# google-research/multinerf

Hardware: NVIDIA H100
Metric: train-step rays/sec @16384 rays x (64+64+32) samples (higher is better)
Workload: dtype bf16

## Files before the change

### multinerf_b200/csrc/gemm_tc.cu

```cuda
#include <cuda.h>

#include <stdlib.h>
#include <string.h>

#include <algorithm>

#include "tc_common.cuh"

namespace mnrf {

constexpr int BLOCK_M = 128;
constexpr int BLOCK_K = 64;
constexpr int A_STAGE_BYTES = BLOCK_M * BLOCK_K * 2;
constexpr int NUM_THREADS = 384;
constexpr int CS_MAX = 1024;
constexpr int gemm_stages(int bn) { return bn == 256 ? 4 : bn == 128 ? 6 : 8; }
constexpr int STAGING_BLOCK_BYTES = 64 * 128;
constexpr int staging_blocks(int mode, int bn, bool ts) {
  return !ts ? 0 : (mode == MNRF_GEMM_FWD && bn >= 128) ? 2 : 1;
}
constexpr int mask_words(int bn) { return bn >= 128 ? bn / 32 : 0; }
constexpr int MASK_BUFS = 2;
constexpr int dgrad_smem_bytes(int bn) { return 8 * bn * 4 + MASK_BUFS * BLOCK_M * mask_words(bn) * 4; }
constexpr int SIDE_SCRATCH = 96 * 8;
// ... 95 lines not shown
      const int64_t col0 = WEIGHTED ? (int64_t)m_blk * BLOCK_M : (int64_t)n_blk * COLS;
      float* out = WEIGHTED ? p.side_aw : p.bsum;
      for (int col = t; col < COLS; col += NT) {
        if (WEIGHTED && col0 + col >= p.m) break;
        float sum = 0.f;
#pragma unroll
        for (int g = 0; g < G; ++g) sum += __uint_as_float(ld_shared_u32(scratch + (g * COLS + col) * 4));
        atomicAdd(out + col0 + col, sum);
      }
    }
  }
}

enum { GK_TURN, GK_FULL, GK_MMA, GK_EPI_LOOP, GK_EPI_SYNC, GK_MASK, GK_N };
#ifdef MNRF_GEMM_CLOCKS
__device__ unsigned long long g_gemm_clk[2][GK_N];
struct GemmClk {
  long long t[GK_N] = {};
  long long last = 0;
  __device__ __forceinline__ void start() { last = clock64(); }
  __device__ __forceinline__ void tick(int k) {
    const long long now = clock64();
    t[k] += now - last;
    last = now;
  }
};
#else
struct GemmClk {
  __device__ __forceinline__ void start() {}
  __device__ __forceinline__ void tick(int) {}
};
#endif

enum { EPI_GENERIC = 0, EPI_BITS_TMA = 1, EPI_BITS_TMA_RANK1 = 2 };

template <int MODE, int NC, bool TS, int SB, bool SMOOTH, int OPS = EPI_GENERIC>
__device__ __forceinline__ void gemm_epilogue(const GemmParams& p, const CUtensorMap* tmap_c, const float (&acc)[NC / 2],
                                              int m_blk, int r0, int ncol0, int wg, uint8_t* smem_c, bool mask_tma,
                                              uint32_t m_tile, bool do_cs, uint32_t cs_lane, int& sblk, GemmClk& clk) {
  constexpr int MW = mask_words(NC);
  static_assert(OPS == EPI_GENERIC || (MODE == MNRF_GEMM_DGRAD && TS && !SMOOTH && MW > 0),
                "fixed operand sets are DGRAD epilogues of the staged store with TMA-loaded mask bits");
  constexpr bool kFixed = OPS != EPI_GENERIC;
  const bool has_rowv = kFixed ? OPS == EPI_BITS_TMA_RANK1 : p.rowv != nullptr;
  const bool has_bits = kFixed || p.maskbits != nullptr;
  const bool bits_tma = kFixed || mask_tma;
  const bool has_mask = !kFixed && p.mask != nullptr;
  const bool has_addend = !kFixed && p.addend != nullptr;
  const int lane = threadIdx.x & 31;
  const int r_in = r0 + (16 * ((threadIdx.x >> 5) & 3) + (lane >> 2));
  const int cq = 2 * (lane & 3);
  const bool leader = (threadIdx.x & 127) == 0;
  const uint32_t c_row = smem_u32(smem_c) + wg * (SB * STAGING_BLOCK_BYTES) + (r_in - r0) * 128 + (cq << 1);
  const uint32_t m_row = m_tile + r_in * (MW * 4);
  int64_t rows[2];
  bool row_ok[2];
  float rv[2] = {0.f, 0.f};
  const uint32_t* mrow[2] = {nullptr, nullptr};
#pragma unroll
  for (int h = 0; h < 2; ++h) {
    rows[h] = (int64_t)m_blk * BLOCK_M + r_in + 8 * h;
    row_ok[h] = rows[h] < p.m;
    if (MODE == MNRF_GEMM_DGRAD && row_ok[h]) {
      if (has_rowv) rv[h] = p.rowv[rows[h]];
      if (has_bits && !bits_tma)
        mrow[h] = p.maskbits + (p.mask_mod > 0 ? rows[h] % p.mask_mod : rows[h]) * p.ldmaskbits;
    }
  }
  uint32_t bits[2] = {0u, 0u};
  uint32_t mw[2] = {0u, 0u};
#pragma unroll
  for (int i = 0; i < NC / 8; ++i) {
    const int col = ncol0 + 8 * i + cq;
    const int sb = SB == 3 ? sblk : (i >> 3) & (SB - 1);
    if (TS && SB == 1 && (i & 7) == 0) {
      clk.tick(GK_EPI_LOOP);
      if (leader) tma_store_wait_read<0>();
      named_bar_sync(2 + wg, 128);
      clk.tick(GK_EPI_SYNC);
    }
    if (MODE == MNRF_GEMM_DGRAD && has_bits && (i & 3) == 0) {
#pragma unroll
      for (int h = 0; h < 2; ++h)
        mw[h] = bits_tma ? ld_shared_u32(m_row + (8 * h * MW + (i >> 2)) * 4)
                         : row_ok[h] ? __ldg(mrow[h] + (col >> 5)) : 0u;
    }
    float v[2][2];
#pragma unroll
    for (int h = 0; h < 2; ++h) { v[h][0] = acc[4 * i + 2 * h]; v[h][1] = acc[4 * i + 2 * h + 1]; }
    if (MODE == MNRF_GEMM_FWD) {
      if (p.bias) {
        const float2 b = __ldg(reinterpret_cast<const float2*>(p.bias + col));
#pragma unroll
        for (int h = 0; h < 2; ++h) { v[h][0] += b.x; v[h][1] += b.y; }
      }
      if constexpr (SMOOTH) {
#pragma unroll
        for (int h = 0; h < 2; ++h) {
          if (p.mask && row_ok[h])
            *reinterpret_cast<uint32_t*>(const_cast<__nv_bfloat16*>(p.mask) + rows[h] * p.ldmask + col) =
                pack_bf16(v[h][0], v[h][1]);
          v[h][0] = act_fwd(p.act, v[h][0]);
          v[h][1] = act_fwd(p.act, v[h][1]);
        }
      } else if (p.act == MNRF_ACT_RELU) {
#pragma unroll
        for (int h = 0; h < 2; ++h)
#pragma unroll
          for (int e = 0; e < 2; ++e) {
            v[h][e] = relu_nan(v[h][e]);
            bits[h] |= (v[h][e] > 0.f ? 1u : 0u) << ((8 * i + cq + e) & 31);
          }
      }
    } else {
      float2 cv = make_float2(0.f, 0.f);
      if (has_rowv) cv = __ldg(reinterpret_cast<const float2*>(p.colv + col));
#pragma unroll
      for (int h = 0; h < 2; ++h) {
        if (has_rowv) { v[h][0] += rv[h] * cv.x; v[h][1] += rv[h] * cv.y; }
        if constexpr (SMOOTH) {
          if (row_ok[h]) {
            const int64_t zr = p.mask_mod > 0 ? rows[h] % p.mask_mod : rows[h];
            const uint32_t zz = __ldg(reinterpret_cast<const unsigned int*>(p.mask + zr * p.ldmask + col));
            v[h][0] *= act_d1(p.act, bf16_lo(zz));
            v[h][1] *= act_d1(p.act, bf16_hi(zz));
          }
        } else if (has_bits) {
          if (!((mw[h] >> (col & 31)) & 1u)) v[h][0] = 0.f;
          if (!((mw[h] >> ((col + 1) & 31)) & 1u)) v[h][1] = 0.f;
        } else if (has_mask && row_ok[h]) {
          const uint32_t mm = __ldg(reinterpret_cast<const unsigned int*>(p.mask + rows[h] * p.ldmask + col));
          if (!(bf16_lo(mm) > 0.f)) v[h][0] = 0.f;
          if (!(bf16_hi(mm) > 0.f)) v[h][1] = 0.f;
        }
        if (has_addend && row_ok[h]) {
          const uint32_t aa = __ldg(reinterpret_cast<const unsigned int*>(p.addend + rows[h] * p.ldadd + col));
          v[h][0] += bf16_lo(aa);
          v[h][1] += bf16_hi(aa);
        }
      }
      if (do_cs) {
        const bool hi = (lane >> 2) & 1;
        const float s0 = v[0][0] + v[1][0], s1 = v[0][1] + v[1][1];
        float t = (hi ? s1 : s0) + __shfl_xor_sync(0xffffffffu, hi ? s0 : s1, 4);
        t += __shfl_xor_sync(0xffffffffu, t, 8);
        t += __shfl_xor_sync(0xffffffffu, t, 16);
        if (lane < 8) {
          const uint32_t a = cs_lane + 8 * i * 4;
          st_shared_u32(a, __float_as_uint(__uint_as_float(ld_shared_u32(a)) + t));
        }
      }
    }
#pragma unroll
    for (int h = 0; h < 2; ++h) {
      if (TS) {
        st_shared_u32(c_row + sb * STAGING_BLOCK_BYTES + h * (8 * 128) + (((i & 7) ^ ((lane >> 2) & 7)) << 4),
                      pack_bf16(v[h][0], v[h][1]));
      } else if (row_ok[h]) {
        *reinterpret_cast<uint32_t*>(reinterpret_cast<__nv_bfloat16*>(p.out) + rows[h] * p.ldc + col) =
            pack_bf16(v[h][0], v[h][1]);
      }
    }
    if (MODE == MNRF_GEMM_FWD && p.act == MNRF_ACT_RELU && p.maskbits && (i & 3) == 3) {
#pragma unroll
      for (int h = 0; h < 2; ++h) {
        bits[h] |= __shfl_xor_sync(0xffffffffu, bits[h], 1);
        bits[h] |= __shfl_xor_sync(0xffffffffu, bits[h], 2);
        if ((lane & 3) == ((i >> 2) & 3) && row_ok[h]) p.maskbits[rows[h] * p.ldmaskbits + (col >> 5)] = bits[h];
        bits[h] = 0u;
      }
    }
    if (TS && (i & 7) == 7) {
      fence_proxy_async();
      clk.tick(GK_EPI_LOOP);
      if (SB >= 2 && leader) tma_store_wait_read<SB - 2>();
      named_bar_sync(2 + wg, 128);
      if (leader) {
        tma_store_2d(tmap_c, smem_c + (wg * SB + sb) * STAGING_BLOCK_BYTES, ncol0 + 8 * (i & ~7),
                     (int)((int64_t)m_blk * BLOCK_M + r0));
        tma_store_commit();
      }
      if (SB == 3) sblk = sblk == 2 ? 0 : sblk + 1;
      clk.tick(GK_EPI_SYNC);
    }
  }
}

template <int MODE, int BN, bool TS, bool SIDE, bool SMOOTH = false>
__global__ void __launch_bounds__(NUM_THREADS, 1)
gemm_tc_kernel(const __grid_constant__ CUtensorMap tmap_a, const __grid_constant__ CUtensorMap tmap_b,
               const __grid_constant__ CUtensorMap tmap_c, const __grid_constant__ CUtensorMap tmap_m,
               const GemmParams p) {
  constexpr int STAGES = gemm_stages(BN);
  constexpr int B_STAGE = BN * BLOCK_K * 2;
  constexpr bool kWgrad = (MODE == MNRF_GEMM_WGRAD);
  constexpr bool kDgrad = (MODE == MNRF_GEMM_DGRAD);
  constexpr int NACC = BN / 2;
  constexpr int SB = staging_blocks(MODE, BN, TS);
  constexpr int MW = mask_words(BN);
  static_assert(SB < 2 || (BN / 64) % 2 == 0, "block j of every tile must use staging block j % SB");
  static_assert(!SIDE || kWgrad, "side sums are a WGRAD feature");
  static_assert(!SMOOTH || (TS && !kWgrad), "smooth activations are FWD / DGRAD epilogues of the staged store");
  extern __shared__ uint8_t smem_dyn[];
  uint8_t* smem = reinterpret_cast<uint8_t*>((reinterpret_cast<uintptr_t>(smem_dyn) + 1023) & ~uintptr_t(1023));
  uint8_t* smem_a = smem;
  uint8_t* smem_b = smem + STAGES * A_STAGE_BYTES;
  uint8_t* smem_c = smem_b + STAGES * B_STAGE;
  float* cs_s = reinterpret_cast<float*>(smem_c + 2 * SB * STAGING_BLOCK_BYTES);
  float* side_s = cs_s;
  uint32_t* mask_s = reinterpret_cast<uint32_t*>(cs_s + (kDgrad ? 8 * BN : SIDE ? SIDE_SCRATCH : 0));
  uint64_t* full_bar = reinterpret_cast<uint64_t*>(mask_s + (kDgrad ? MASK_BUFS * BLOCK_M * MW : 0));
  uint64_t* empty_bar = full_bar + STAGES;
// ... 130 lines not shown
      int sblk = 0;
      GemmClk clk;
      clk.start();
      gemm_epilogue<MODE, BN, TS, SB, SMOOTH>(p, &tmap_c, acc, m_blk, 64 * c, ncol0, c, smem_c, mask_tma,
                                              smem_u32(mask_s) + (it % MASK_BUFS) * (BLOCK_M * MW * 4), do_cs, cs_lane,
                                              sblk, clk);
      if (mask_tma) {
        __syncwarp();
        if (lane == 0) mbar_arrive(&mask_empty[it % MASK_BUFS]);
      }
      const int next = tile + (int)gridDim.x;
      if (do_cs && (next >= total_tiles || next % p.num_n_blocks != n_blk)) {
        named_bar_sync(1, 2 * 128);
        for (int j = threadIdx.x - 128; j < BN; j += 2 * 128) {
          float s = 0.f;
#pragma unroll
          for (int sw = 0; sw < 8; ++sw) {
            s += cs_s[sw * BN + j];
            cs_s[sw * BN + j] = 0.f;
          }
          atomicAdd(p.colsum + ncol0 + j, s);
        }
        named_bar_sync(1, 2 * 128);
      }
    }
    if (TS && (threadIdx.x & 127) == 0) tma_store_wait_all();
  }
}

constexpr int PP_BN = 128;
constexpr int PP_STAGES = 5;
constexpr int pp_staging_blocks(int mode) { return mode == MNRF_GEMM_DGRAD ? 3 : 2; }
constexpr int PP_MASK_BUFS = 4;
constexpr int pp_smem_bytes(int mode) {
  return PP_STAGES * (A_STAGE_BYTES + PP_BN * BLOCK_K * 2) + 2 * pp_staging_blocks(mode) * STAGING_BLOCK_BYTES +
         (mode == MNRF_GEMM_DGRAD ? PP_MASK_BUFS * BLOCK_M * mask_words(PP_BN) * 4 : 0) + 256  +
         1024 ;
}

template <int MODE, int BN, int OPS>
__global__ void __launch_bounds__(NUM_THREADS, 1)
gemm_tc_pingpong_kernel(const __grid_constant__ CUtensorMap tmap_a, const __grid_constant__ CUtensorMap tmap_b,
                        const __grid_constant__ CUtensorMap tmap_c, const __grid_constant__ CUtensorMap tmap_m,
                        const GemmParams p) {
  constexpr int STAGES = PP_STAGES;
  constexpr int B_STAGE = PP_BN * BLOCK_K * 2;
  constexpr int SUB = BN / PP_BN;
  constexpr int MW = mask_words(PP_BN);
  constexpr int SB = pp_staging_blocks(MODE);
  constexpr bool kDgrad = (MODE == MNRF_GEMM_DGRAD);
  static_assert(MODE != MNRF_GEMM_WGRAD && (BN == 128 || BN == 256), "FWD / DGRAD tiles of 128 or 256 columns");
  extern __shared__ uint8_t smem_dyn[];
  uint8_t* smem = reinterpret_cast<uint8_t*>((reinterpret_cast<uintptr_t>(smem_dyn) + 1023) & ~uintptr_t(1023));
  uint8_t* smem_a = smem;
  uint8_t* smem_b = smem + STAGES * A_STAGE_BYTES;
  uint8_t* smem_c = smem_b + STAGES * B_STAGE;
  uint32_t* mask_s = reinterpret_cast<uint32_t*>(smem_c + 2 * SB * STAGING_BLOCK_BYTES);
  uint64_t* full_bar = reinterpret_cast<uint64_t*>(mask_s + (kDgrad ? PP_MASK_BUFS * BLOCK_M * MW : 0));
  uint64_t* empty_bar = full_bar + STAGES;
  uint64_t* mask_full = empty_bar + STAGES;
  uint64_t* mask_empty = mask_full + PP_MASK_BUFS;
  uint64_t* mma_turn = mask_empty + PP_MASK_BUFS;

  const int lane = threadIdx.x & 31;
  const int wg = threadIdx.x >> 7;
  const int total_tiles = p.num_m_blocks * p.num_n_blocks;
  const int nk = p.num_k_blocks;
  const bool mask_tma = kDgrad && (OPS != EPI_GENERIC || p.mask_tma);

  if (threadIdx.x == 0) {
    prefetch_tmap(&tmap_a);
    prefetch_tmap(&tmap_b);
    prefetch_tmap(&tmap_c);
    if (mask_tma) prefetch_tmap(&tmap_m);
    for (int i = 0; i < STAGES; ++i) {
      mbar_init(&full_bar[i], 1);
      mbar_init(&empty_bar[i], 4);
    }
    for (int i = 0; i < PP_MASK_BUFS; ++i) {
      mbar_init(&mask_full[i], 1);
      mbar_init(&mask_empty[i], 4);
    }
    for (int i = 0; i < 2; ++i) mbar_init(&mma_turn[i], 4);
    fence_barrier_init();
  }
  __syncthreads();
  pdl_launch_dependents();
  pdl_wait();

  if (wg == 0) {
    setmaxnreg_dec<40>();
    if (threadIdx.x == 0) {
      uint32_t stage = 0, phase = 0;
      int it = 0;
      for (int tile = blockIdx.x; tile < total_tiles; tile += gridDim.x) {
        const int n_blk = tile % p.num_n_blocks;
        const int m_blk = tile / p.num_n_blocks;
        for (int s = 0; s < SUB; ++s, ++it) {
          const int ncol0 = n_blk * BN + s * PP_BN;
          if (mask_tma) {
            const int mb = it % PP_MASK_BUFS;
            mbar_wait(&mask_empty[mb], ((it / PP_MASK_BUFS) & 1) ^ 1, 4);
            mbar_expect_tx(&mask_full[mb], BLOCK_M * MW * 4);
            const int64_t r0 = (int64_t)m_blk * BLOCK_M;
            tma_load_2d(mask_s + mb * (BLOCK_M * MW), &tmap_m, &mask_full[mb], ncol0 / 32,
                        (int)(p.mask_mod > 0 ? r0 % p.mask_mod : r0));
          }
          for (int kb = 0; kb < nk; ++kb) {
            mbar_wait(&empty_bar[stage], phase ^ 1, 1);
            mbar_expect_tx(&full_bar[stage], A_STAGE_BYTES + B_STAGE);
            tma_load_2d(smem_a + stage * A_STAGE_BYTES, &tmap_a, &full_bar[stage], kb * BLOCK_K, m_blk * BLOCK_M);
            tma_load_2d(smem_b + stage * B_STAGE, &tmap_b, &full_bar[stage], kb * BLOCK_K, ncol0);
            if (++stage == STAGES) { stage = 0; phase ^= 1; }
          }
        }
      }
    }
  } else {
    setmaxnreg_inc<232>();
    const int c = wg - 1;
    float acc[2][64];
    int sblk = 0;
    GemmClk clk;
    clk.start();
    for (int it = c; ; it += 2) {
      const int tile = blockIdx.x + (it / SUB) * (int)gridDim.x;
      if (tile >= total_tiles) break;
      const int s = it % SUB;
      const int n_blk = tile % p.num_n_blocks;
      const int m_blk = tile / p.num_n_blocks;
      const int ncol0 = n_blk * BN + s * PP_BN;
      const uint32_t slot = (uint32_t)it * (uint32_t)nk;
      uint32_t stage = slot % STAGES, phase = (slot / STAGES) & 1;
      clk.tick(GK_EPI_LOOP);
      if (it > 0) mbar_wait(&mma_turn[c], ((it - 1) >> 1) & 1, 7);
      clk.tick(GK_TURN);
      int prev = -1;
      fence_acc(acc[0]);
      fence_acc(acc[1]);
      for (int kb = 0; kb < nk; ++kb) {
        mbar_wait(&full_bar[stage], phase, 3);
        clk.tick(GK_FULL);
        const uint32_t sa = smem_u32(smem_a + stage * A_STAGE_BYTES);
        const uint32_t sb = smem_u32(smem_b + stage * B_STAGE);
        wgmma_fence();
#pragma unroll
        for (int k = 0; k < BLOCK_K / WGMMA_K; ++k) {
          const uint64_t bdesc = make_smem_desc(sb + k * (WGMMA_K * 2), 0, 1024);
#pragma unroll
          for (int g = 0; g < 2; ++g)
            Wgmma<PP_BN, 0, 0>::mma(acc[g], make_smem_desc(sa + g * (64 * 128) + k * (WGMMA_K * 2), 0, 1024), bdesc,
                                    (kb > 0 || k > 0) ? 1u : 0u);
        }
        wgmma_commit();
        wgmma_wait<1>();
        if (prev >= 0 && lane == 0) mbar_arrive(&empty_bar[prev]);
        prev = (int)stage;
        if (++stage == STAGES) { stage = 0; phase ^= 1; }
        clk.tick(GK_MMA);
      }
      if (blockIdx.x + ((it + 1) / SUB) * (int)gridDim.x < total_tiles) {
        __syncwarp();
        if (lane == 0) mbar_arrive(&mma_turn[c ^ 1]);
      }
      wgmma_wait<0>();
      fence_acc(acc[0]);
      fence_acc(acc[1]);
      if (prev >= 0 && lane == 0) mbar_arrive(&empty_bar[prev]);
      clk.tick(GK_MMA);

      const uint32_t m_base = smem_u32(mask_s) + (it % PP_MASK_BUFS) * (BLOCK_M * MW * 4);
      if (mask_tma) mbar_wait(&mask_full[it % PP_MASK_BUFS], (it / PP_MASK_BUFS) & 1, 5);
      clk.tick(GK_MASK);
#pragma unroll 1
      for (int g = 0; g < 2; ++g) {
        gemm_epilogue<MODE, PP_BN, true, SB, false, OPS>(p, &tmap_c, acc[0], m_blk, 64 * g, ncol0, c, smem_c, mask_tma,
                                                         m_base, false, 0, sblk, clk);
#pragma unroll
        for (int e = 0; e < 64; ++e) acc[0][e] = acc[1][e];
      }
      if (mask_tma) {
        __syncwarp();
        if (lane == 0) mbar_arrive(&mask_empty[it % PP_MASK_BUFS]);
      }
    }
    if ((threadIdx.x & 127) == 0) tma_store_wait_all();
#ifdef MNRF_GEMM_CLOCKS
    clk.tick(GK_EPI_SYNC);
    if (blockIdx.x == 0 && (threadIdx.x & 127) == 0)
      for (int k = 0; k < GK_N; ++k) atomicAdd(&g_gemm_clk[c][k], (unsigned long long)clk.t[k]);
#endif
  }
}

template <int MODE, int BN, int OPS = EPI_GENERIC>
static int launch_gemm_tc_pingpong(int grid, const CUtensorMap& ta, const CUtensorMap& tb, const CUtensorMap& tc,
                                   const CUtensorMap& tm, const GemmParams& p, cudaStream_t stream) {
  constexpr int kSmem = pp_smem_bytes(MODE);
  static_assert(kSmem <= 232448, "shared memory budget");
  return launch_tc<gemm_tc_pingpong_kernel<MODE, BN, OPS>>(grid, NUM_THREADS, kSmem, stream, ta, tb, tc, tm, p);
}

template <int BN>
static int launch_dgrad_pingpong(int ops, int grid, const CUtensorMap& ta, const CUtensorMap& tb, const CUtensorMap& tc,
                                 const CUtensorMap& tm, const GemmParams& p, cudaStream_t stream) {
  switch (ops) {
    case EPI_BITS_TMA:
      return launch_gemm_tc_pingpong<MNRF_GEMM_DGRAD, BN, EPI_BITS_TMA>(grid, ta, tb, tc, tm, p, stream);
    case EPI_BITS_TMA_RANK1:
      return launch_gemm_tc_pingpong<MNRF_GEMM_DGRAD, BN, EPI_BITS_TMA_RANK1>(grid, ta, tb, tc, tm, p, stream);
  }
  return launch_gemm_tc_pingpong<MNRF_GEMM_DGRAD, BN>(grid, ta, tb, tc, tm, p, stream);
}

template <int MODE, int BN, bool TS, bool SIDE, bool SMOOTH = false>
static int launch_gemm_tc(int grid, const CUtensorMap& ta, const CUtensorMap& tb, const CUtensorMap& tc,
                          const CUtensorMap& tm, const GemmParams& p, cudaStream_t stream) {
  constexpr int kSmem = smem_bytes(MODE, BN, TS, SIDE);
  static_assert(kSmem <= 232448, "shared memory budget");
  return launch_tc<gemm_tc_kernel<MODE, BN, TS, SIDE, SMOOTH>>(grid, NUM_THREADS, kSmem, stream, ta, tb, tc, tm, p);
}

int gemm_tc_smooth_launch(int mode, int block_n, int grid, const CUtensorMap& ta, const CUtensorMap& tb,
                          const CUtensorMap& tc, const GemmParams& p, cudaStream_t stream);

#ifndef MNRF_GEMM_TC_SMOOTH_UNIT
static int pick_block_n(int n) {
  const int cands[] = {256, 128, 64, 32, 16};
  for (int c : cands)
    if (n % c == 0) return c;
  return 0;
}

static int gemm_tc_plan(const mnrf_gemm_desc* d, const mnrf_bf16* a, const mnrf_bf16* b, const float* bias,
                        const float* colv, const mnrf_bf16* mask, const uint32_t* maskbits, const float* colsum,
                        const mnrf_bf16* addend, const void* out, const float* bsum, const float* side_w,
                        const float* side_aw, const mnrf_bf16* z, int64_t ldz, mnrf_gemm_instance* plan,
                        GemmParams* p) {
  MNRF_CHECK(d->mode == MNRF_GEMM_WGRAD || d->k % BLOCK_K == 0,
             "mnrf_gemm(tc): reduction length %d must be a multiple of %d", d->k, BLOCK_K);
  MNRF_CHECK(d->lda % 8 == 0 && d->ldb % 8 == 0 && ((uintptr_t)a % 16) == 0 && ((uintptr_t)b % 16) == 0,
             "mnrf_gemm(tc): operands must be 16-byte aligned with ld %% 8 == 0");
  const int block_n = pick_block_n(d->n);
  MNRF_CHECK(block_n > 0, "mnrf_gemm(tc): N=%d must be a multiple of 16", d->n);
  if (d->mode == MNRF_GEMM_WGRAD)
// ... 15 lines not shown
    MNRF_CHECK(!maskbits && !mask, "mnrf_gemm(tc): a smooth activation takes z, not a ReLU mask");
    MNRF_CHECK(d->mode == MNRF_GEMM_FWD || z, "mnrf_gemm(tc): the DGRAD of a smooth activation needs z");
    MNRF_CHECK(!z || (ldz % 2 == 0 && ((uintptr_t)z % 4) == 0), "mnrf_gemm(tc): z must be 4-byte aligned");
  }
  if (bias) MNRF_CHECK(((uintptr_t)bias % 8) == 0, "mnrf_gemm(tc): bias must be 8-byte aligned");
  if (colv) MNRF_CHECK(((uintptr_t)colv % 8) == 0, "mnrf_gemm(tc): colv must be 8-byte aligned");
  const int workers = mnrf_num_sms();
  const int num_m_blocks = (int)((d->m + BLOCK_M - 1) / BLOCK_M);
  const int num_n_blocks = d->n / block_n;
  const int num_k_blocks = (d->k + BLOCK_K - 1) / BLOCK_K;
  int num_splits = 1;
  if (d->mode == MNRF_GEMM_WGRAD) {
    const int out_tiles = num_m_blocks * num_n_blocks;
    const int max_splits = std::min(std::max(1, (2 * workers) / out_tiles), num_k_blocks);
    int splits = max_splits;
    for (int sp = 1; sp <= max_splits; ++sp) {
      const int items = out_tiles * sp;
      const int rounds = (items + workers - 1) / workers;
      if (items * 100 >= rounds * workers * 95) { splits = sp; break; }
    }
    num_splits = splits;
  }
  const int kblocks_per_split = (num_k_blocks + num_splits - 1) / num_splits;
  num_splits = (num_k_blocks + kblocks_per_split - 1) / kblocks_per_split;
  if (d->mode != MNRF_GEMM_WGRAD) {
    MNRF_CHECK(d->ldc % 2 == 0 && ((uintptr_t)out % 4) == 0, "mnrf_gemm(tc): bf16 output must be 4-byte aligned");
    if (mask) MNRF_CHECK(d->ldmask % 2 == 0 && ((uintptr_t)mask % 4) == 0, "mnrf_gemm(tc): mask must be 4-byte aligned");
  } else {
    MNRF_CHECK(d->ldc % 2 == 0 && ((uintptr_t)out % 8) == 0, "mnrf_gemm(tc): fp32 output must be 8-byte aligned");
  }
  const bool ts = d->mode != MNRF_GEMM_WGRAD && block_n >= 64 && ((uintptr_t)out % 16) == 0 && d->ldc % 8 == 0;
  MNRF_CHECK(!smooth || ts, "mnrf_gemm(tc): a smooth activation needs N %% 64 == 0 and a 16-byte aligned output "
             "with a row pitch that is a multiple of 8");
  const bool mask_tma = d->mode == MNRF_GEMM_DGRAD && maskbits && mask_words(block_n) > 0 && d->ldmaskbits % 4 == 0 &&
                        ((uintptr_t)maskbits % 16) == 0 && (d->mask_mod == 0 || d->mask_mod % BLOCK_M == 0);
  const bool pingpong = d->mode != MNRF_GEMM_WGRAD && ts && d->n % PP_BN == 0 && !smooth && !colsum;
  int epilogue = EPI_GENERIC;
  if (pingpong && d->mode == MNRF_GEMM_DGRAD && mask_tma && !mask && !addend)
    epilogue = colv ? EPI_BITS_TMA_RANK1 : EPI_BITS_TMA;
  const int tiles = num_m_blocks * num_n_blocks * num_splits;
  plan->block_n = block_n;
  plan->staged = ts;
  plan->mask_tma = mask_tma;
  plan->smooth = smooth;
  plan->side = side;
  plan->splits = num_splits;
  plan->tiles = tiles;
  plan->grid = std::min(tiles, workers);
  plan->pingpong = pingpong;
  plan->epilogue = epilogue;
  p->num_m_blocks = num_m_blocks;
  p->num_n_blocks = num_n_blocks;
  p->num_k_blocks = num_k_blocks;
  p->num_splits = num_splits;
  p->kblocks_per_split = kblocks_per_split;
  return 0;
}

template <int MODE>
static int launch_register_store(int block_n, int grid, const CUtensorMap& ta, const CUtensorMap& tb,
                                 const CUtensorMap& tc, const CUtensorMap& tm, const GemmParams& p,
                                 cudaStream_t stream) {
  switch (block_n) {
    case 256: return launch_gemm_tc<MODE, 256, false, false>(grid, ta, tb, tc, tm, p, stream);
    case 128: return launch_gemm_tc<MODE, 128, false, false>(grid, ta, tb, tc, tm, p, stream);
    case 64: return launch_gemm_tc<MODE, 64, false, false>(grid, ta, tb, tc, tm, p, stream);
    case 32: return launch_gemm_tc<MODE, 32, false, false>(grid, ta, tb, tc, tm, p, stream);
    case 16: return launch_gemm_tc<MODE, 16, false, false>(grid, ta, tb, tc, tm, p, stream);
  }
  set_error("mnrf_gemm(tc): no register-store instance at BN=%d", block_n);
  return 1;
}

static int launch_gemm_tc_plan(int mode, const mnrf_gemm_instance& plan, const CUtensorMap& ta, const CUtensorMap& tb,
                               const CUtensorMap& tc, const CUtensorMap& tm, const GemmParams& p,
                               cudaStream_t stream) {
  const int bn = plan.block_n, grid = plan.grid;
  const bool fwd = mode == MNRF_GEMM_FWD;
  if (plan.pingpong) {
    if (bn == 256)
      return fwd ? launch_gemm_tc_pingpong<MNRF_GEMM_FWD, 256>(grid, ta, tb, tc, tm, p, stream)
                 : launch_dgrad_pingpong<256>(plan.epilogue, grid, ta, tb, tc, tm, p, stream);
    if (bn == 128)
      return fwd ? launch_gemm_tc_pingpong<MNRF_GEMM_FWD, 128>(grid, ta, tb, tc, tm, p, stream)
                 : launch_dgrad_pingpong<128>(plan.epilogue, grid, ta, tb, tc, tm, p, stream);
  } else if (plan.smooth) {
    return gemm_tc_smooth_launch(mode, bn, grid, ta, tb, tc, p, stream);
  } else if (mode == MNRF_GEMM_WGRAD) {
    if (bn == 256)
      return plan.side ? launch_gemm_tc<MNRF_GEMM_WGRAD, 256, false, true>(grid, ta, tb, tc, tm, p, stream)
                       : launch_gemm_tc<MNRF_GEMM_WGRAD, 256, false, false>(grid, ta, tb, tc, tm, p, stream);
    if (bn == 128)
      return plan.side ? launch_gemm_tc<MNRF_GEMM_WGRAD, 128, false, true>(grid, ta, tb, tc, tm, p, stream)
                       : launch_gemm_tc<MNRF_GEMM_WGRAD, 128, false, false>(grid, ta, tb, tc, tm, p, stream);
    if (bn == 64)
      return plan.side ? launch_gemm_tc<MNRF_GEMM_WGRAD, 64, false, true>(grid, ta, tb, tc, tm, p, stream)
                       : launch_gemm_tc<MNRF_GEMM_WGRAD, 64, false, false>(grid, ta, tb, tc, tm, p, stream);
  } else if (!plan.staged) {
    return fwd ? launch_register_store<MNRF_GEMM_FWD>(bn, grid, ta, tb, tc, tm, p, stream)
               : launch_register_store<MNRF_GEMM_DGRAD>(bn, grid, ta, tb, tc, tm, p, stream);
  } else if (bn == 64) {
    return fwd ? launch_gemm_tc<MNRF_GEMM_FWD, 64, true, false>(grid, ta, tb, tc, tm, p, stream)
               : launch_gemm_tc<MNRF_GEMM_DGRAD, 64, true, false>(grid, ta, tb, tc, tm, p, stream);
  } else if (!fwd) {
    if (bn == 256) return launch_gemm_tc<MNRF_GEMM_DGRAD, 256, true, false>(grid, ta, tb, tc, tm, p, stream);
    if (bn == 128) return launch_gemm_tc<MNRF_GEMM_DGRAD, 128, true, false>(grid, ta, tb, tc, tm, p, stream);
  }
  set_error("mnrf_gemm(tc): no kernel instance for mode %d, BN=%d, staged %d, side sums %d", mode, bn, plan.staged,
            plan.side);
  return 1;
}

int gemm_tc_launch(const mnrf_gemm_desc* d, const mnrf_bf16* a, const mnrf_bf16* b, const float* bias,
                   const float* rowv, const float* colv, const mnrf_bf16* mask, uint32_t* maskbits,
                   float* colsum, const mnrf_bf16* addend, void* out, cudaStream_t stream, float* bsum,
                   const float* side_w, float* side_aw, mnrf_bf16* z, int64_t ldz) {
  mnrf_gemm_instance plan;
// ... 5 lines not shown
  const bool ts = plan.staged;
  p.mode = d->mode; p.act = d->act; p.m = d->m; p.n = d->n; p.k = d->k;
  p.ldc = d->ldc; p.ldmask = d->ldmask;
  p.bias = bias; p.rowv = rowv; p.colv = colv;
  p.mask = reinterpret_cast<const __nv_bfloat16*>(mask);
  p.out = out;
  p.maskbits = maskbits;
  p.ldmaskbits = d->ldmaskbits;
  p.mask_mod = d->mask_mod;
  p.addend = reinterpret_cast<const __nv_bfloat16*>(addend);
  p.ldadd = d->ldadd;
  p.colsum = colsum;
  p.bsum = bsum; p.side_w = side_w; p.side_aw = side_aw;
  if (plan.smooth) {
    p.mask = reinterpret_cast<const __nv_bfloat16*>(z);
    p.ldmask = ldz;
  }
  p.mask_tma = plan.mask_tma;
  CUtensorMap ta, tb, tc;
  if (d->mode != MNRF_GEMM_WGRAD) {
    if (make_tmap(&ta, a, d->m, d->k, d->lda, BLOCK_K, BLOCK_M)) return 1;
    if (make_tmap(&tb, b, d->n, d->k, d->ldb, BLOCK_K, plan.pingpong ? PP_BN : block_n)) return 1;
  } else {
    if (make_tmap(&ta, a, d->k, d->m, d->lda, 64, BLOCK_K)) return 1;
    if (make_tmap(&tb, b, d->k, d->n, d->ldb, 64, BLOCK_K)) return 1;
  }
  if (ts) {
    if (make_tmap(&tc, out, d->m, d->n, d->ldc, 64, 64)) return 1;
  } else {
    tc = tb;
  }
  CUtensorMap tm = tb;
  if (p.mask_tma &&
      make_tmap(&tm, maskbits, d->mask_mod > 0 ? d->mask_mod : d->m, d->n / 32, d->ldmaskbits,
                mask_words(plan.pingpong ? PP_BN : block_n), BLOCK_M, CU_TENSOR_MAP_DATA_TYPE_UINT32, 4,
                CU_TENSOR_MAP_SWIZZLE_NONE))
    return 1;
  if (plan.grid == 0) return 0;
  if (int rc = launch_gemm_tc_plan(d->mode, plan, ta, tb, tc, tm, p, stream)) return rc;
  MNRF_LAUNCH_CHECK();
  return 0;
}
#endif

}

#ifndef MNRF_GEMM_TC_SMOOTH_UNIT
extern "C" int mnrf_gemm_plan(const mnrf_gemm_desc* d, const mnrf_bf16* a, const mnrf_bf16* b, const float* bias,
                              const float* rowv, const float* colv, const mnrf_bf16* mask, const uint32_t* maskbits,
                              const float* colsum, const mnrf_bf16* addend, const mnrf_bf16* z, int64_t ldz,
                              const void* out, const float* bsum, const float* side_w, const float* side_aw,
                              mnrf_gemm_instance* plan) {
  MNRF_CHECK(d && plan, "mnrf_gemm_plan: null pointer");
  MNRF_CHECK((rowv == nullptr) == (colv == nullptr), "mnrf_gemm: rowv and colv come together");
  MNRF_CHECK(!mask || d->mask_mod == 0, "mnrf_gemm: mask_mod applies to maskbits and z, not to a bf16 mask");
  mnrf::GemmParams p;
  return mnrf::gemm_tc_plan(d, a, b, bias, colv, mask, maskbits, colsum, addend, out, bsum, side_w, side_aw, z, ldz,
                            plan, &p);
}

#ifdef MNRF_GEMM_CLOCKS
extern "C" int mnrf_gemm_clocks(unsigned long long* out) {
  unsigned long long zero[2 * mnrf::GK_N] = {};
  if (cudaDeviceSynchronize() != cudaSuccess) return 1;
  if (cudaMemcpyFromSymbol(out, mnrf::g_gemm_clk, sizeof(zero)) != cudaSuccess) return 1;
  return cudaMemcpyToSymbol(mnrf::g_gemm_clk, zero, sizeof(zero)) != cudaSuccess;
}
// ... 3 lines not shown
```

### multinerf_b200/csrc/tc_common.cuh

```cuda
#pragma once

#include <cuda.h>
#include <stdlib.h>

#include "common.cuh"
#include "wgmma.cuh"

namespace mnrf {

constexpr int WGMMA_K = 16;

__device__ __forceinline__ uint32_t smem_u32(const void* p) {
  return static_cast<uint32_t>(__cvta_generic_to_shared(p));
}
__device__ __forceinline__ void mbar_init(uint64_t* bar, uint32_t count) {
  asm volatile("mbarrier.init.shared::cta.b64 [%0], %1;" ::"r"(smem_u32(bar)), "r"(count));
}
__device__ __forceinline__ void mbar_expect_tx(uint64_t* bar, uint32_t bytes) {
  asm volatile("mbarrier.arrive.expect_tx.shared::cta.b64 _, [%0], %1;" ::"r"(smem_u32(bar)), "r"(bytes) : "memory");
}
__device__ __forceinline__ void mbar_arrive(uint64_t* bar) {
  asm volatile("mbarrier.arrive.shared::cta.b64 _, [%0];" ::"r"(smem_u32(bar)) : "memory");
}
__device__ __forceinline__ bool mbar_try_wait(uint64_t* bar, uint32_t parity) {
// ... 2 lines not shown
      "{\n"
      ".reg .pred p;\n"
      "mbarrier.try_wait.parity.shared::cta.b64 p, [%1], %2;\n"
      "selp.u32 %0, 1, 0, p;\n"
      "}\n"
      : "=r"(ok) : "r"(smem_u32(bar)), "r"(parity) : "memory");
  return ok != 0;
}
__device__ __forceinline__ void mbar_wait(uint64_t* bar, uint32_t parity, int tag) {
  (void)tag;
  if (mbar_try_wait(bar, parity)) return;
  const long long t0 = clock64();
  while (!mbar_try_wait(bar, parity)) {
    if (clock64() - t0 > 4000000000LL) __trap();
  }
}
__device__ __forceinline__ void fence_barrier_init() {
  asm volatile("fence.mbarrier_init.release.cluster;" ::: "memory");
}
__device__ __forceinline__ void fence_proxy_async() {
  asm volatile("fence.proxy.async.shared::cta;" ::: "memory");
}
__device__ __forceinline__ void tma_load_2d(void* smem_dst, const CUtensorMap* map, uint64_t* bar,
                                            int c0, int c1) {
  asm volatile(
      "cp.async.bulk.tensor.2d.shared::cluster.global.mbarrier::complete_tx::bytes [%0], [%1, {%3, %4}], [%2];"
      :: "r"(smem_u32(smem_dst)), "l"(reinterpret_cast<uint64_t>(map)), "r"(smem_u32(bar)), "r"(c0), "r"(c1)
      : "memory");
}
__device__ __forceinline__ void tma_prefetch_2d(const CUtensorMap* map, int c0, int c1) {
  asm volatile("cp.async.bulk.prefetch.tensor.2d.L2.global.tile [%0, {%1, %2}];"
               :: "l"(reinterpret_cast<uint64_t>(map)), "r"(c0), "r"(c1) : "memory");
}
__device__ __forceinline__ void tma_store_2d(const CUtensorMap* map, const void* smem_src, int c0, int c1) {
  asm volatile("cp.async.bulk.tensor.2d.global.shared::cta.bulk_group [%0, {%2, %3}], [%1];"
               :: "l"(reinterpret_cast<uint64_t>(map)), "r"(smem_u32(smem_src)), "r"(c0), "r"(c1) : "memory");
}
__device__ __forceinline__ void tma_store_commit() { asm volatile("cp.async.bulk.commit_group;" ::: "memory"); }
template <int N>
__device__ __forceinline__ void tma_store_wait_read() {
  asm volatile("cp.async.bulk.wait_group.read %0;" ::"n"(N) : "memory");
}
__device__ __forceinline__ void tma_store_wait_all() { asm volatile("cp.async.bulk.wait_group 0;" ::: "memory"); }
__device__ __forceinline__ void prefetch_tmap(const CUtensorMap* map) {
  asm volatile("prefetch.tensormap [%0];" ::"l"(reinterpret_cast<uint64_t>(map)) : "memory");
}
__device__ __forceinline__ void st_shared_u32(uint32_t addr, uint32_t v) {
  asm volatile("st.shared.b32 [%0], %1;" ::"r"(addr), "r"(v) : "memory");
}
__device__ __forceinline__ uint32_t ld_shared_u32(uint32_t addr) {
  uint32_t v;
  asm volatile("ld.shared.b32 %0, [%1];" : "=r"(v) : "r"(addr) : "memory");
  return v;
}
__device__ __forceinline__ uint4 ld_shared_v4(uint32_t addr) {
  uint4 v;
  asm volatile("ld.shared.v4.b32 {%0, %1, %2, %3}, [%4];"
               : "=r"(v.x), "=r"(v.y), "=r"(v.z), "=r"(v.w) : "r"(addr) : "memory");
  return v;
}
__device__ __forceinline__ void named_bar_sync(int id, int count) {
  asm volatile("bar.sync %0, %1;" ::"r"(id), "r"(count) : "memory");
}

template <int R>
__device__ __forceinline__ void setmaxnreg_dec() { asm volatile("setmaxnreg.dec.sync.aligned.u32 %0;" ::"n"(R)); }
template <int R>
__device__ __forceinline__ void setmaxnreg_inc() { asm volatile("setmaxnreg.inc.sync.aligned.u32 %0;" ::"n"(R)); }

__device__ __forceinline__ void wgmma_fence() { asm volatile("wgmma.fence.sync.aligned;" ::: "memory"); }
__device__ __forceinline__ void wgmma_commit() { asm volatile("wgmma.commit_group.sync.aligned;" ::: "memory"); }
template <int N>
__device__ __forceinline__ void wgmma_wait() { asm volatile("wgmma.wait_group.sync.aligned %0;" ::"n"(N) : "memory"); }
template <int R>
__device__ __forceinline__ void fence_acc(float (&d)[R]) {
#pragma unroll
  for (int i = 0; i < R; ++i) asm volatile("" : "+f"(d[i])::"memory");
}
__device__ __forceinline__ void pdl_wait() { asm volatile("griddepcontrol.wait;" ::: "memory"); }
__device__ __forceinline__ void pdl_launch_dependents() { asm volatile("griddepcontrol.launch_dependents;" ::: "memory"); }

__device__ __forceinline__ uint64_t make_smem_desc(uint32_t saddr, uint32_t lbo_bytes, uint32_t sbo_bytes) {
  uint64_t d = 0;
  d |= (uint64_t)((saddr >> 4) & 0x3fff);
  d |= (uint64_t)((lbo_bytes >> 4) & 0x3fff) << 16;
// ... 66 lines not shown
```

### multinerf_b200/models.py

```python
import dataclasses
import math
import os
from typing import Any, Dict, List, Optional

import numpy as np
import torch

from . import configs
from . import geopoly
from . import lib as L
from . import ops
from . import utils


def _pad64(n):
  return (n + 63) // 64 * 64


@dataclasses.dataclass
class DenseSpec:
  name: str
  role: str
  in_dim: int
  in_pad: int
# ... 488 lines not shown
      st.raw_rgb, st.d_raw_rgb = st.raw_head.view(B, S, 4)[..., 1:], st.d_raw_head.view(B, S, 4)[..., 1:]
    elif plan.top == 'view':
      Wv = cfg.net_width_viewdirs
      nv = cfg.net_depth_viewdirs
      st.vacts = [torch.empty(M, Wv + plan.vin_pad if i in plan.view_concat_after else Wv, device=dev, dtype=bf)
                  for i in range(nv)]
      if relu:
        st.vbits = [torch.empty(M, Wv // 32, device=dev, dtype=torch.int32) for _ in range(nv)]
      else:
        st.vzs = [torch.empty(M, Wv, device=dev, dtype=bf) for _ in range(nv)]
      if plan.view_concat_after:
        st.vin = st.vacts[plan.view_concat_after[0]][:, Wv:]
        st.vin_copies = [st.vacts[i][:, Wv:] for i in plan.view_concat_after[1:]]
      else:
        st.vin = torch.empty(M, plan.vin_pad, device=dev, dtype=bf)
      st.raw_rgb = torch.empty(B, S, 3, device=dev)
      st.d_raw_rgb = torch.empty(B, S, 3, device=dev)
    for sp in plan.narrow:
      st.heads[sp.role] = torch.empty(M, sp.out_dim, device=dev)
      st.d_heads[sp.role] = torch.empty(M, sp.out_dim, device=dev)
    if plan.has_normals_stage:
      if plan.pred_normals:
        st.normals_pred = torch.empty(M, 3, device=dev)
      if plan.ref_stage and cfg.enable_pred_roughness:
        st.roughness = torch.empty(M, device=dev)
      st.extra_dw = torch.empty(B, S, device=dev)
    if keep:
      self._levels[key] = st
    return st

  @staticmethod
  def _act_out(plan, st, i, view=False):
    if plan.act == L.ACT_RELU:
      return dict(act=L.ACT_RELU, maskbits=(st.vbits if view else st.bits)[i])
    return dict(act=plan.act, z=(st.vzs if view else st.zs)[i] if st.keep_acts else None)

  @staticmethod
  def _act_grad(plan, st, i, view=False, head=False):
    if plan.act == L.ACT_RELU:
      return dict(relu_mask=True) if head else dict(maskbits=(st.vbits if view else st.bits)[i])
    return dict(act=plan.act, z=(st.vzs if view else st.zs)[i])

  def _refdir_args(self, st, mlp, viewdirs):
    plan = mlp.plan
    cfg = plan.cfg
    mat, ml, ide_n = mlp.ide or (None, None, 0)
    desc = ops.refdir_desc(
        st.M, st.S, use_pred_normals=plan.pred_normals, use_density_normals=plan.density_normals,
        use_reflections=cfg.use_reflections, use_ide=cfg.use_directional_enc, use_n_dot_v=cfg.use_n_dot_v,
        use_roughness=cfg.enable_pred_roughness, deg_view=cfg.deg_view, ide_n=ide_n,
        roughness_bias=cfg.roughness_bias, ld=st.vin.stride(0), col0=plan.enc_col0, col_end=plan.vin_pad)
    return desc, mat, ml, st.heads.get('grad_pred'), st.heads.get('roughness'), st.rgd, viewdirs

  def _mlp_forward(self, st: LevelState, mlp: MLPDevice, rays, impl=0, loss_mults=None):
    plan = mlp.plan
    cfg = plan.cfg
    m = self.mcfg
    ops.encode(st.sdist, rays.origins, rays.directions, rays.radii_flat, rays.near_flat,
               rays.far_flat, mlp.basis, min_deg=cfg.min_deg_point, max_deg=cfg.max_deg_point,
               raydist_fn=m.raydist_fn, ray_shape=m.ray_shape, warp_contract=cfg.warp_fn == 'contract',
               disable_integration=m.disable_integration, feat=st.feat, feat_cols=plan.Fpad, tfeat=st.tfeat)
    self._mlp_stages(st, mlp, rays.viewdirs, impl, loss_mults)

  def _mlp_stages(self, st, mlp, viewdirs, impl=0, loss_mults=None):
    plan = mlp.plan
    self._trunk_layers(st, mlp, impl)
    if plan.density_normals:
# ... 562 lines not shown
```

Before: 284,600.

## Specialize forward pingpong GEMM epilogues with smem bias and TMA-stored relu mask bits

Adds compile-time fixed forward epilogue variants (bias+relu+bits, bias+relu, bias) for the pingpong GEMM kernel. Bias is staged once per tile into shared memory instead of per-element global loads. Relu mask words go to shared memory and are written out with a single TMA store rather than scattered global stores. In models.py, mask bits are skipped when activations are not kept, which removes redundant bit writes in no-grad passes. The cost is more template instantiations and some extra shared memory and sync per tile.

```diff
diff --git a/multinerf_b200/csrc/gemm_tc.cu b/multinerf_b200/csrc/gemm_tc.cu
--- a/multinerf_b200/csrc/gemm_tc.cu
+++ b/multinerf_b200/csrc/gemm_tc.cu
@@ -151,21 +151,29 @@
 };
 #endif
 
-enum { EPI_GENERIC = 0, EPI_BITS_TMA = 1, EPI_BITS_TMA_RANK1 = 2 };
+enum {
+  EPI_GENERIC = 0, EPI_BITS_TMA = 1, EPI_BITS_TMA_RANK1 = 2,
+  EPI_FWD_BIAS_RELU_BITS = 3, EPI_FWD_BIAS_RELU = 4, EPI_FWD_BIAS = 5
+};
+constexpr bool epi_fwd(int ops) { return ops >= EPI_FWD_BIAS_RELU_BITS; }
 
 template <int MODE, int NC, bool TS, int SB, bool SMOOTH, int OPS = EPI_GENERIC>
 __device__ __forceinline__ void gemm_epilogue(const GemmParams& p, const CUtensorMap* tmap_c, const float (&acc)[NC / 2],
                                               int m_blk, int r0, int ncol0, int wg, uint8_t* smem_c, bool mask_tma,
-                                              uint32_t m_tile, bool do_cs, uint32_t cs_lane, int& sblk, GemmClk& clk) {
+                                              uint32_t m_tile, bool do_cs, uint32_t cs_lane, int& sblk, GemmClk& clk,
+                                              const CUtensorMap* tmap_m = nullptr, uint32_t bias_s = 0) {
   constexpr int MW = mask_words(NC);
-  static_assert(OPS == EPI_GENERIC || (MODE == MNRF_GEMM_DGRAD && TS && !SMOOTH && MW > 0),
-                "fixed operand sets are DGRAD epilogues of the staged store with TMA-loaded mask bits");
+  static_assert(OPS == EPI_GENERIC || ((MODE == MNRF_GEMM_FWD) == epi_fwd(OPS) && TS && !SMOOTH && MW > 0),
+                "fixed operand sets are FWD / DGRAD epilogues of the staged store with mask words by TMA");
   constexpr bool kFixed = OPS != EPI_GENERIC;
+  constexpr bool kFwdFixed = kFixed && epi_fwd(OPS);
   const bool has_rowv = kFixed ? OPS == EPI_BITS_TMA_RANK1 : p.rowv != nullptr;
-  const bool has_bits = kFixed || p.maskbits != nullptr;
+  const bool has_bits = kFixed ? OPS == EPI_FWD_BIAS_RELU_BITS || !kFwdFixed : p.maskbits != nullptr;
   const bool bits_tma = kFixed || mask_tma;
   const bool has_mask = !kFixed && p.mask != nullptr;
   const bool has_addend = !kFixed && p.addend != nullptr;
+  const bool has_bias = kFixed || p.bias != nullptr;
+  const bool relu = kFixed ? OPS != EPI_FWD_BIAS : p.act == MNRF_ACT_RELU;
   const int lane = threadIdx.x & 31;
   const int r_in = r0 + (16 * ((threadIdx.x >> 5) & 3) + (lane >> 2));
   const int cq = 2 * (lane & 3);
@@ -208,8 +216,9 @@
 #pragma unroll
     for (int h = 0; h < 2; ++h) { v[h][0] = acc[4 * i + 2 * h]; v[h][1] = acc[4 * i + 2 * h + 1]; }
     if (MODE == MNRF_GEMM_FWD) {
-      if (p.bias) {
-        const float2 b = __ldg(reinterpret_cast<const float2*>(p.bias + col));
+      if (has_bias) {
+        const float2 b = kFwdFixed ? ld_shared_f2(bias_s + (8 * i + cq) * 4)
+                                   : __ldg(reinterpret_cast<const float2*>(p.bias + col));
 #pragma unroll
         for (int h = 0; h < 2; ++h) { v[h][0] += b.x; v[h][1] += b.y; }
       }
@@ -222,13 +231,13 @@
           v[h][0] = act_fwd(p.act, v[h][0]);
           v[h][1] = act_fwd(p.act, v[h][1]);
         }
-      } else if (p.act == MNRF_ACT_RELU) {
+      } else if (relu) {
 #pragma unroll
         for (int h = 0; h < 2; ++h)
 #pragma unroll
           for (int e = 0; e < 2; ++e) {
             v[h][e] = relu_nan(v[h][e]);
-            bits[h] |= (v[h][e] > 0.f ? 1u : 0u) << ((8 * i + cq + e) & 31);
+            bits[h] |= (v[h][e] > 0.f ? 1u : 0u) << (8 * (i & 3) + e);
           }
       }
     } else {
@@ -280,12 +289,16 @@
             pack_bf16(v[h][0], v[h][1]);
       }
     }
-    if (MODE == MNRF_GEMM_FWD && p.act == MNRF_ACT_RELU && p.maskbits && (i & 3) == 3) {
+    if (MODE == MNRF_GEMM_FWD && relu && has_bits && (i & 3) == 3) {
 #pragma unroll
       for (int h = 0; h < 2; ++h) {
+        bits[h] <<= cq;
         bits[h] |= __shfl_xor_sync(0xffffffffu, bits[h], 1);
         bits[h] |= __shfl_xor_sync(0xffffffffu, bits[h], 2);
-        if ((lane & 3) == ((i >> 2) & 3) && row_ok[h]) p.maskbits[rows[h] * p.ldmaskbits + (col >> 5)] = bits[h];
+        if ((lane & 3) == ((i >> 2) & 3)) {
+          if (kFwdFixed) st_shared_u32(m_row + (8 * h * MW + (i >> 2)) * 4, bits[h]);
+          else if (row_ok[h]) p.maskbits[rows[h] * p.ldmaskbits + (col >> 5)] = bits[h];
+        }
         bits[h] = 0u;
       }
     }
@@ -297,6 +310,8 @@
       if (leader) {
         tma_store_2d(tmap_c, smem_c + (wg * SB + sb) * STAGING_BLOCK_BYTES, ncol0 + 8 * (i & ~7),
                      (int)((int64_t)m_blk * BLOCK_M + r0));
+        if (OPS == EPI_FWD_BIAS_RELU_BITS && i == NC / 8 - 1 && r0 == BLOCK_M - 64)
+          tma_store_2d(tmap_m, m_tile, ncol0 / 32, m_blk * BLOCK_M);
         tma_store_commit();
       }
       if (SB == 3) sblk = sblk == 2 ? 0 : sblk + 1;
@@ -493,10 +508,11 @@
 constexpr int PP_STAGES = 5;
 constexpr int pp_staging_blocks(int mode) { return mode == MNRF_GEMM_DGRAD ? 3 : 2; }
 constexpr int PP_MASK_BUFS = 4;
-constexpr int pp_smem_bytes(int mode) {
+constexpr int pp_smem_bytes(int mode, int ops) {
   return PP_STAGES * (A_STAGE_BYTES + PP_BN * BLOCK_K * 2) + 2 * pp_staging_blocks(mode) * STAGING_BLOCK_BYTES +
-         (mode == MNRF_GEMM_DGRAD ? PP_MASK_BUFS * BLOCK_M * mask_words(PP_BN) * 4 : 0) + 256  +
-         1024 ;
+         (mode == MNRF_GEMM_DGRAD || ops == EPI_FWD_BIAS_RELU_BITS ? PP_MASK_BUFS * BLOCK_M * mask_words(PP_BN) * 4
+                                                                   : 0) +
+         (epi_fwd(ops) ? 2 * PP_BN * 4 : 0) + 256  + 1024 ;
 }
 
 template <int MODE, int BN, int OPS>
@@ -510,6 +526,8 @@
   constexpr int MW = mask_words(PP_BN);
   constexpr int SB = pp_staging_blocks(MODE);
   constexpr bool kDgrad = (MODE == MNRF_GEMM_DGRAD);
+  constexpr bool kFwdFixed = epi_fwd(OPS);
+  constexpr bool kFwdBits = OPS == EPI_FWD_BIAS_RELU_BITS;
   static_assert(MODE != MNRF_GEMM_WGRAD && (BN == 128 || BN == 256), "FWD / DGRAD tiles of 128 or 256 columns");
   extern __shared__ uint8_t smem_dyn[];
   uint8_t* smem = reinterpret_cast<uint8_t*>((reinterpret_cast<uintptr_t>(smem_dyn) + 1023) & ~uintptr_t(1023));
@@ -517,7 +535,8 @@
   uint8_t* smem_b = smem + STAGES * A_STAGE_BYTES;
   uint8_t* smem_c = smem_b + STAGES * B_STAGE;
   uint32_t* mask_s = reinterpret_cast<uint32_t*>(smem_c + 2 * SB * STAGING_BLOCK_BYTES);
-  uint64_t* full_bar = reinterpret_cast<uint64_t*>(mask_s + (kDgrad ? PP_MASK_BUFS * BLOCK_M * MW : 0));
+  float* bias_s = reinterpret_cast<float*>(mask_s + (kDgrad || kFwdBits ? PP_MASK_BUFS * BLOCK_M * MW : 0));
+  uint64_t* full_bar = reinterpret_cast<uint64_t*>(bias_s + (kFwdFixed ? 2 * PP_BN : 0));
   uint64_t* empty_bar = full_bar + STAGES;
   uint64_t* mask_full = empty_bar + STAGES;
   uint64_t* mask_empty = mask_full + PP_MASK_BUFS;
@@ -533,7 +552,7 @@
     prefetch_tmap(&tmap_a);
     prefetch_tmap(&tmap_b);
     prefetch_tmap(&tmap_c);
-    if (mask_tma) prefetch_tmap(&tmap_m);
+    if (mask_tma || kFwdBits) prefetch_tmap(&tmap_m);
     for (int i = 0; i < STAGES; ++i) {
       mbar_init(&full_bar[i], 1);
       mbar_init(&empty_bar[i], 4);
@@ -591,6 +610,7 @@
       const int n_blk = tile % p.num_n_blocks;
       const int m_blk = tile / p.num_n_blocks;
       const int ncol0 = n_blk * BN + s * PP_BN;
+      const float bias_v = kFwdFixed ? __ldg(p.bias + ncol0 + (threadIdx.x & 127)) : 0.f;
       const uint32_t slot = (uint32_t)it * (uint32_t)nk;
       uint32_t stage = slot % STAGES, phase = (slot / STAGES) & 1;
       clk.tick(GK_EPI_LOOP);
@@ -632,11 +652,16 @@
 
       const uint32_t m_base = smem_u32(mask_s) + (it % PP_MASK_BUFS) * (BLOCK_M * MW * 4);
       if (mask_tma) mbar_wait(&mask_full[it % PP_MASK_BUFS], (it / PP_MASK_BUFS) & 1, 5);
+      const uint32_t bias_wg = smem_u32(bias_s) + c * (PP_BN * 4);
+      if (kFwdFixed) {
+        st_shared_u32(bias_wg + (threadIdx.x & 127) * 4, __float_as_uint(bias_v));
+        named_bar_sync(2 + c, 128);
+      }
       clk.tick(GK_MASK);
 #pragma unroll 1
       for (int g = 0; g < 2; ++g) {
         gemm_epilogue<MODE, PP_BN, true, SB, false, OPS>(p, &tmap_c, acc[0], m_blk, 64 * g, ncol0, c, smem_c, mask_tma,
-                                                         m_base, false, 0, sblk, clk);
+                                                         m_base, false, 0, sblk, clk, &tmap_m, bias_wg);
 #pragma unroll
         for (int e = 0; e < 64; ++e) acc[0][e] = acc[1][e];
       }
@@ -657,7 +682,7 @@
 template <int MODE, int BN, int OPS = EPI_GENERIC>
 static int launch_gemm_tc_pingpong(int grid, const CUtensorMap& ta, const CUtensorMap& tb, const CUtensorMap& tc,
                                    const CUtensorMap& tm, const GemmParams& p, cudaStream_t stream) {
-  constexpr int kSmem = pp_smem_bytes(MODE);
+  constexpr int kSmem = pp_smem_bytes(MODE, OPS);
   static_assert(kSmem <= 232448, "shared memory budget");
   return launch_tc<gemm_tc_pingpong_kernel<MODE, BN, OPS>>(grid, NUM_THREADS, kSmem, stream, ta, tb, tc, tm, p);
 }
@@ -672,6 +697,20 @@
       return launch_gemm_tc_pingpong<MNRF_GEMM_DGRAD, BN, EPI_BITS_TMA_RANK1>(grid, ta, tb, tc, tm, p, stream);
   }
   return launch_gemm_tc_pingpong<MNRF_GEMM_DGRAD, BN>(grid, ta, tb, tc, tm, p, stream);
+}
+
+template <int BN>
+static int launch_fwd_pingpong(int ops, int grid, const CUtensorMap& ta, const CUtensorMap& tb, const CUtensorMap& tc,
+                               const CUtensorMap& tm, const GemmParams& p, cudaStream_t stream) {
+  switch (ops) {
+    case EPI_FWD_BIAS_RELU_BITS:
+      return launch_gemm_tc_pingpong<MNRF_GEMM_FWD, BN, EPI_FWD_BIAS_RELU_BITS>(grid, ta, tb, tc, tm, p, stream);
+    case EPI_FWD_BIAS_RELU:
+      return launch_gemm_tc_pingpong<MNRF_GEMM_FWD, BN, EPI_FWD_BIAS_RELU>(grid, ta, tb, tc, tm, p, stream);
+    case EPI_FWD_BIAS:
+      return launch_gemm_tc_pingpong<MNRF_GEMM_FWD, BN, EPI_FWD_BIAS>(grid, ta, tb, tc, tm, p, stream);
+  }
+  return launch_gemm_tc_pingpong<MNRF_GEMM_FWD, BN>(grid, ta, tb, tc, tm, p, stream);
 }
 
 template <int MODE, int BN, bool TS, bool SIDE, bool SMOOTH = false>
@@ -753,12 +792,20 @@
   const bool ts = d->mode != MNRF_GEMM_WGRAD && block_n >= 64 && ((uintptr_t)out % 16) == 0 && d->ldc % 8 == 0;
   MNRF_CHECK(!smooth || ts, "mnrf_gemm(tc): a smooth activation needs N %% 64 == 0 and a 16-byte aligned output "
              "with a row pitch that is a multiple of 8");
-  const bool mask_tma = d->mode == MNRF_GEMM_DGRAD && maskbits && mask_words(block_n) > 0 && d->ldmaskbits % 4 == 0 &&
-                        ((uintptr_t)maskbits % 16) == 0 && (d->mask_mod == 0 || d->mask_mod % BLOCK_M == 0);
+  const bool bits_tma_ok = maskbits && mask_words(block_n) > 0 && d->ldmaskbits % 4 == 0 &&
+                           ((uintptr_t)maskbits % 16) == 0;
+  bool mask_tma = d->mode == MNRF_GEMM_DGRAD && bits_tma_ok && (d->mask_mod == 0 || d->mask_mod % BLOCK_M == 0);
   const bool pingpong = d->mode != MNRF_GEMM_WGRAD && ts && d->n % PP_BN == 0 && !smooth && !colsum;
   int epilogue = EPI_GENERIC;
   if (pingpong && d->mode == MNRF_GEMM_DGRAD && mask_tma && !mask && !addend)
     epilogue = colv ? EPI_BITS_TMA_RANK1 : EPI_BITS_TMA;
+  if (pingpong && d->mode == MNRF_GEMM_FWD && bias) {
+    if (d->act == MNRF_ACT_RELU)
+      epilogue = !maskbits ? EPI_FWD_BIAS_RELU : bits_tma_ok ? EPI_FWD_BIAS_RELU_BITS : EPI_GENERIC;
+    else if (d->act == MNRF_ACT_NONE && !maskbits)
+      epilogue = EPI_FWD_BIAS;
+    mask_tma = epilogue == EPI_FWD_BIAS_RELU_BITS;
+  }
   const int tiles = num_m_blocks * num_n_blocks * num_splits;
   plan->block_n = block_n;
   plan->staged = ts;
@@ -800,10 +847,10 @@
   const bool fwd = mode == MNRF_GEMM_FWD;
   if (plan.pingpong) {
     if (bn == 256)
-      return fwd ? launch_gemm_tc_pingpong<MNRF_GEMM_FWD, 256>(grid, ta, tb, tc, tm, p, stream)
+      return fwd ? launch_fwd_pingpong<256>(plan.epilogue, grid, ta, tb, tc, tm, p, stream)
                  : launch_dgrad_pingpong<256>(plan.epilogue, grid, ta, tb, tc, tm, p, stream);
     if (bn == 128)
-      return fwd ? launch_gemm_tc_pingpong<MNRF_GEMM_FWD, 128>(grid, ta, tb, tc, tm, p, stream)
+      return fwd ? launch_fwd_pingpong<128>(plan.epilogue, grid, ta, tb, tc, tm, p, stream)
                  : launch_dgrad_pingpong<128>(plan.epilogue, grid, ta, tb, tc, tm, p, stream);
   } else if (plan.smooth) {
     return gemm_tc_smooth_launch(mode, bn, grid, ta, tb, tc, p, stream);
@@ -875,7 +922,8 @@
   }
   CUtensorMap tm = tb;
   if (p.mask_tma &&
-      make_tmap(&tm, maskbits, d->mask_mod > 0 ? d->mask_mod : d->m, d->n / 32, d->ldmaskbits,
+      make_tmap(&tm, maskbits, d->mode == MNRF_GEMM_DGRAD && d->mask_mod > 0 ? d->mask_mod : d->m, d->n / 32,
+                d->ldmaskbits,
                 mask_words(plan.pingpong ? PP_BN : block_n), BLOCK_M, CU_TENSOR_MAP_DATA_TYPE_UINT32, 4,
                 CU_TENSOR_MAP_SWIZZLE_NONE))
     return 1;
diff --git a/multinerf_b200/csrc/tc_common.cuh b/multinerf_b200/csrc/tc_common.cuh
--- a/multinerf_b200/csrc/tc_common.cuh
+++ b/multinerf_b200/csrc/tc_common.cuh
@@ -58,9 +58,12 @@
   asm volatile("cp.async.bulk.prefetch.tensor.2d.L2.global.tile [%0, {%1, %2}];"
                :: "l"(reinterpret_cast<uint64_t>(map)), "r"(c0), "r"(c1) : "memory");
 }
+__device__ __forceinline__ void tma_store_2d(const CUtensorMap* map, uint32_t smem_src, int c0, int c1) {
+  asm volatile("cp.async.bulk.tensor.2d.global.shared::cta.bulk_group [%0, {%2, %3}], [%1];"
+               :: "l"(reinterpret_cast<uint64_t>(map)), "r"(smem_src), "r"(c0), "r"(c1) : "memory");
+}
 __device__ __forceinline__ void tma_store_2d(const CUtensorMap* map, const void* smem_src, int c0, int c1) {
-  asm volatile("cp.async.bulk.tensor.2d.global.shared::cta.bulk_group [%0, {%2, %3}], [%1];"
-               :: "l"(reinterpret_cast<uint64_t>(map)), "r"(smem_u32(smem_src)), "r"(c0), "r"(c1) : "memory");
+  tma_store_2d(map, smem_u32(smem_src), c0, c1);
 }
 __device__ __forceinline__ void tma_store_commit() { asm volatile("cp.async.bulk.commit_group;" ::: "memory"); }
 template <int N>
@@ -77,6 +80,11 @@
 __device__ __forceinline__ uint32_t ld_shared_u32(uint32_t addr) {
   uint32_t v;
   asm volatile("ld.shared.b32 %0, [%1];" : "=r"(v) : "r"(addr) : "memory");
+  return v;
+}
+__device__ __forceinline__ float2 ld_shared_f2(uint32_t addr) {
+  float2 v;
+  asm volatile("ld.shared.v2.f32 {%0, %1}, [%2];" : "=f"(v.x), "=f"(v.y) : "r"(addr) : "memory");
   return v;
 }
 __device__ __forceinline__ uint4 ld_shared_v4(uint32_t addr) {
diff --git a/multinerf_b200/models.py b/multinerf_b200/models.py
--- a/multinerf_b200/models.py
+++ b/multinerf_b200/models.py
@@ -544,7 +544,7 @@
   @staticmethod
   def _act_out(plan, st, i, view=False):
     if plan.act == L.ACT_RELU:
-      return dict(act=L.ACT_RELU, maskbits=(st.vbits if view else st.bits)[i])
+      return dict(act=L.ACT_RELU, maskbits=(st.vbits if view else st.bits)[i] if st.keep_acts else None)
     return dict(act=plan.act, z=(st.vzs if view else st.zs)[i] if st.keep_acts else None)
 
   @staticmethod
```

After: 293,500 (median of 6 runs). 3.1% higher.
